# facebookresearch/esm

Measured on AMD Instinct MI355X. Metric: residues/sec (whole node) ESM-2 650M L=1022 bulk extract, higher is better.
Workload: dtype f16; 1 GPU; esm2_t33_650M_UR50D forward (repr_layers=[33] + logits), synthetic tokens [B,1024], random-init weights of the 650M architecture; batch_per_gpu=64, seq_len=1022, ln_fold=on (library default)

## Files before the change

esm_amd/csrc/gemm9.hip:

```cpp
#include "gemm_epi.h"
#include <type_traits>

namespace esmk {

constexpr int Q_BUF = 65536;
constexpr int Q_WOFF = 32768;
constexpr int Q_EPI = 2 * Q_BUF;
constexpr int Q_SLICE = 8192;
constexpr int Q_LDS = Q_EPI + 4 * Q_SLICE;

#define ESMK_INL __attribute__((always_inline))

template <typename T, int EPI, bool FULL, int D = 4, bool NT = true, int NMI = 8, bool SB = false, bool LNF = false>
ESMK_DEV void epilogue9_f32(const GemmArgs& p, f32x4 (&acc)[8][NMI], int m_base, int n_base, int lane, char* wl) {
    static_assert(!LNF || EPI == EPI_RESID_F32, "the LayerNorm-fold producer is the residual epilogue");
    constexpr bool lnp = LNF;
    constexpr int NP = 2 * NMI;
    constexpr int NIB = NMI / 2;
    float s1[4], s2[4];
    float cmv[2][4];
    typedef unsigned u32x2 __attribute__((ext_vector_type(2)));
    typedef unsigned u32x4 __attribute__((ext_vector_type(4)));
    u32x2 hold[4];
    T* h16 = reinterpret_cast<T*>(p.h16);
    if constexpr (!FULL)
        if (n_base >= p.N || m_base >= p.M) return;
    float* out = reinterpret_cast<float*>(p.out);
    const int ldc = p.N;
    const int g4 = lane >> 4, l16 = lane & 15;
    f32x4 old[D][4];
    auto load_old = [&](f32x4 (&dst)[4], int piece) ESMK_INL {
        const int i = piece >> 2, jb = piece & 3;
#pragma unroll
        for (int it = 0; it < 4; ++it) {
            const int pc = it * 64 + lane;
            const int m = FULL ? m_base + 32 * i + (pc >> 3) : min(m_base + 32 * i + (pc >> 3), p.M - 1);
            const int n = FULL ? n_base + 32 * jb + (pc & 7) * 4 : min(n_base + 32 * jb + (pc & 7) * 4, p.N - 4);
            dst[it] = *reinterpret_cast<const f32x4*>(out + (size_t)m * ldc + n);
        }
    };
    if constexpr (EPI == EPI_RESID_F32) {
#pragma unroll
        for (int d = 0; d < D; ++d) load_old(old[d], d);
    }
    auto load_means = [&](int i) ESMK_INL {
#pragma unroll
        for (int it = 0; it < 4; ++it) {
            const int m = m_base + 32 * i + it * 8 + (lane >> 3);
            cmv[i & 1][it] = (kExperiments && (p.lnf_dbg & 4)) ? 0.f : p.ln_mean[FULL ? m : min(m, p.M - 1)];
        }
    };
    if constexpr (LNF)
        if (lnp) load_means(0);
#pragma unroll
    for (int piece = 0; piece < NP; ++piece) {
        const int i = piece >> 2, jb = piece & 3;
        char* sl = wl + (SB ? 0 : (piece & 1) * 4096);
        if constexpr (LNF) {
            if (jb == 0 && lnp) {
#pragma unroll
                for (int it = 0; it < 4; ++it) s1[it] = s2[it] = 0.f;
                if (i + 1 < NIB) load_means(i + 1);
            }
        }
#pragma unroll
        for (int q = 0; q < 4; ++q) {
            const int mi2 = q >> 1, nj2 = q & 1;
            const int row = 16 * mi2 + l16;
            f32x4 v = acc[2 * jb + nj2][2 * i + mi2];
            if constexpr (EPI == EPI_GELU_F32) gelu_fast_x4(v);
            *reinterpret_cast<f32x4*>(sl + row * 128 + (((4 * nj2 + g4) ^ (row & 7)) << 4)) = v;
        }
        f32x4 vv[4];
#pragma unroll
        for (int it = 0; it < 4; ++it) {
            const int pc = it * 64 + lane;
            const int r = pc >> 3, cc = pc & 7;
            vv[it] = *reinterpret_cast<const f32x4*>(sl + r * 128 + ((cc ^ (r & 7)) << 4));
        }
#pragma unroll
        for (int it = 0; it < 4; ++it) {
            const int pc = it * 64 + lane;
            const int r = pc >> 3, cc = pc & 7;
            f32x4 v = vv[it];
            if constexpr (EPI == EPI_RESID_F32) {
                const f32x4 o = old[piece % D][it];
                v = f32x4{o[0] + v[0], o[1] + v[1], o[2] + v[2], o[3] + v[3]};
            }
            const int m = m_base + 32 * i + r, n = n_base + 32 * jb + cc * 4;
            const bool inside = FULL || (m < p.M && n < p.N);
            if (inside) {
                if constexpr (NT) __builtin_nontemporal_store(v, reinterpret_cast<f32x4*>(out + (size_t)m * ldc + n));
                else *reinterpret_cast<f32x4*>(out + (size_t)m * ldc + n) = v;
            }
            if (LNF && lnp) {
                const float c = cmv[i & 1][it];
                float d0 = v[0] - c, d1 = v[1] - c, d2 = v[2] - c, d3 = v[3] - c;
                if (!inside) d0 = d1 = d2 = d3 = 0.f;
                s1[it] += (d0 + d1) + (d2 + d3);
                s2[it] = __builtin_fmaf(d3, d3, __builtin_fmaf(d2, d2, __builtin_fmaf(d1, d1, __builtin_fmaf(d0, d0, s2[it]))));
                typename Op<T>::v4 pk;
                pk[0] = Op<T>::from(d0), pk[1] = Op<T>::from(d1), pk[2] = Op<T>::from(d2), pk[3] = Op<T>::from(d3);
                const u32x2 cur = __builtin_bit_cast(u32x2, pk);
                if ((jb & 1) == 0) {
                    hold[it] = cur;
                } else {
                    const bool odd = (lane & 1) != 0;
                    const u32x2 prev = hold[it];
                    const u32x2 send = odd ? prev : cur;
                    u32x2 recv;
                    recv.x = (unsigned)__builtin_amdgcn_update_dpp(0, (int)send.x, 0xB1, 0xf, 0xf, true);
                    recv.y = (unsigned)__builtin_amdgcn_update_dpp(0, (int)send.y, 0xB1, 0xf, 0xf, true);
                    const u32x4 o = odd ? u32x4{recv.x, recv.y, cur.x, cur.y} : u32x4{prev.x, prev.y, recv.x, recv.y};
                    const int col = n_base + (odd ? 32 * jb + 4 * (cc - 1) : 32 * (jb - 1) + 4 * cc);
                    if ((FULL || (m < p.M && col < p.N)) && !(kExperiments && (p.lnf_dbg & 1))) {
                        auto* hd = reinterpret_cast<u32x4*>(h16 + (size_t)m * p.ldh + col);
                        if constexpr (NT) __builtin_nontemporal_store(o, hd);
                        else *hd = o;
                    }
                }
            }
        }
        if constexpr (EPI == EPI_RESID_F32)
            if (piece + D < NP) load_old(old[piece % D], piece + D);
        if constexpr (LNF) {
            if (jb == 3 && lnp && !(kExperiments && (p.lnf_dbg & 2))) {
#pragma unroll
                for (int it = 0; it < 4; ++it) {
                    float a = s1[it], b = s2[it];
                    a += __builtin_bit_cast(float, __builtin_amdgcn_update_dpp(0, __builtin_bit_cast(int, a), 0x111, 0xf, 0xf, true));
                    b += __builtin_bit_cast(float, __builtin_amdgcn_update_dpp(0, __builtin_bit_cast(int, b), 0x111, 0xf, 0xf, true));
                    a += __builtin_bit_cast(float, __builtin_amdgcn_update_dpp(0, __builtin_bit_cast(int, a), 0x112, 0xf, 0xf, true));
                    b += __builtin_bit_cast(float, __builtin_amdgcn_update_dpp(0, __builtin_bit_cast(int, b), 0x112, 0xf, 0xf, true));
                    a += __builtin_bit_cast(float, __builtin_amdgcn_update_dpp(0, __builtin_bit_cast(int, a), 0x114, 0xf, 0xf, true));
                    b += __builtin_bit_cast(float, __builtin_amdgcn_update_dpp(0, __builtin_bit_cast(int, b), 0x114, 0xf, 0xf, true));
                    const int m = m_base + 32 * i + it * 8 + (lane >> 3);
                    if ((lane & 7) == 7 && (FULL || m < p.M)) {
                        f32x2 st = {a, b};
                        *reinterpret_cast<f32x2*>(p.ln_part + ((size_t)m * p.ln_parts + (n_base >> 7)) * 2) = st;
                    }
                }
            }
        }
    }
}

template <typename T, int EPI, bool FULL, bool NT = false, int NMI = 8, int RR = 32, bool LNF = false, bool X3O = false>
ESMK_DEV void epilogue9_t(const GemmArgs& p, f32x4 (&acc)[8][NMI], int m_base, int n_base, int lane, char* wl) {
    static_assert(!X3O || (EPI == EPI_GELU_T && !LNF), "hi | hi | lo output rows: the plain GELU epilogue");
    using V8 = typename Op<T>::v8;
    float bs1[8], bs2[8];
    constexpr int LPR = EPI == EPI_QKV_ROPE ? 4 : 8;
    constexpr int RPI = 64 / LPR;
    constexpr int NIT = RR / RPI;
    constexpr int NI_ = NMI * 16 / RR;
    float rsv[LNF ? NI_ : 1][NIT];
    if constexpr (LNF) {
        if (FULL || m_base < p.M) {
#pragma unroll
            for (int i = 0; i < NI_; ++i)
#pragma unroll
                for (int it = 0; it < NIT; ++it) {
                    const int m = m_base + RR * i + RPI * it + lane / LPR;
                    rsv[i][it] = p.ln_rstd[FULL ? m : min(m, p.M - 1)];
                }
        }
    }
    constexpr int NI = NMI * 16 / RR;
    constexpr int NR = 2 * NI;
    constexpr int MB = RR / 16;
    const int g4 = lane >> 4, l16 = lane & 15;
    if constexpr (!FULL)
        if (m_base >= p.M) return;
    auto write_round = [&](int r) ESMK_INL {
        const int hf = r / NI, i = r % NI;
#pragma unroll
        for (int mi2 = 0; mi2 < MB; ++mi2)
#pragma unroll
            for (int nq = 0; nq < 4; ++nq) {
                const int row = 16 * mi2 + l16, chunk = 4 * nq + g4;
                *reinterpret_cast<f32x4*>(wl + row * 256 + ((chunk ^ (row & 7)) << 4)) = acc[4 * hf + nq][MB * i + mi2];
            }
    };
    auto read_round = [&](f32x4 (&raw)[8]) ESMK_INL {
        if constexpr (EPI == EPI_QKV_ROPE) {
#pragma unroll
            for (int it = 0; it < RR / 16; ++it) {
                const int slot = it * 64 + lane;
                const int r = slot >> 2, g4 = slot & 3;
#pragma unroll
                for (int e2 = 0; e2 < 2; ++e2) {
                    raw[4 * it + e2] = *reinterpret_cast<const f32x4*>(wl + r * 256 + (((2 * g4 + e2) ^ (r & 7)) << 4));
                    raw[4 * it + 2 + e2] = *reinterpret_cast<const f32x4*>(wl + r * 256 + (((8 + 2 * g4 + e2) ^ (r & 7)) << 4));
                }
            }
        } else {
#pragma unroll
            for (int it = 0; it < RR / 8; ++it) {
                const int slot = it * 64 + lane;
                const int r = slot >> 3, c8 = slot & 7;
#pragma unroll
                for (int e2 = 0; e2 < 2; ++e2)
                    raw[2 * it + e2] = *reinterpret_cast<const f32x4*>(wl + r * 256 + (((2 * c8 + e2) ^ (r & 7)) << 4));
            }
        }
    };
    auto finish_round = [&](int rd, const f32x4 (&raw)[8]) ESMK_INL {
        const int hf = rd / NI, i = rd % NI;
        const int nb = n_base + 64 * hf;
        if constexpr (!FULL)
            if (nb >= p.N) return;
        if constexpr (EPI == EPI_QKV_ROPE) {
            const int which = nb / p.E;
            const int head = (nb - which * p.E) >> 6;
            T* qk = reinterpret_cast<T*>(which == 0 ? p.q : p.k);
            const float sc = which == 0 ? p.scaling : 1.0f;
            if constexpr (LNF) {
                if (i == 0) {
                    const int c0 = nb + 8 * (lane & 3);
#pragma unroll
                    for (int e2 = 0; e2 < 2; ++e2) {
                        f32x4 a = *reinterpret_cast<const f32x4*>(p.bias + c0 + 4 * e2), b = *reinterpret_cast<const f32x4*>(p.bias + c0 + 32 + 4 * e2);
                        if (p.bias2 != nullptr) {
                            const f32x4 a2 = *reinterpret_cast<const f32x4*>(p.bias2 + c0 + 4 * e2), b2 = *reinterpret_cast<const f32x4*>(p.bias2 + c0 + 32 + 4 * e2);
#pragma unroll
                            for (int e = 0; e < 4; ++e) a[e] += a2[e], b[e] += b2[e];
                        }
#pragma unroll
                        for (int e = 0; e < 4; ++e) bs1[4 * e2 + e] = a[e] * sc, bs2[4 * e2 + e] = b[e] * sc;
                    }
                }
            }
#pragma unroll
            for (int it = 0; it < RR / 16; ++it) {
                const int slot = it * 64 + lane;
                const int r = slot >> 2, g4 = slot & 3;
                const int mm = m_base + RR * i + r;
                const int m = FULL ? mm : min(mm, p.M - 1);
                const int b = m / p.T;
                const int tt = p.row_pos != nullptr ? p.row_pos[m] : m - b * p.T;
                float rs = sc;
                if constexpr (LNF) rs = rsv[i][it] * sc;
                float y1[8], y2[8];
#pragma unroll
                for (int e2 = 0; e2 < 2; ++e2) {
                    const f32x4 c = *reinterpret_cast<const f32x4*>(p.cos + (size_t)tt * 32 + 8 * g4 + 4 * e2);
                    const f32x4 s = *reinterpret_cast<const f32x4*>(p.sin + (size_t)tt * 32 + 8 * g4 + 4 * e2);
#pragma unroll
                    for (int e = 0; e < 4; ++e) {
                        const float x1 = LNF ? __builtin_fmaf(raw[4 * it + e2][e], rs, bs1[4 * e2 + e]) : raw[4 * it + e2][e] * sc;
                        const float x2 = LNF ? __builtin_fmaf(raw[4 * it + 2 + e2][e], rs, bs2[4 * e2 + e]) : raw[4 * it + 2 + e2][e] * sc;
                        y1[4 * e2 + e] = __builtin_fmaf(x1, c[e], -(x2 * s[e]));
                        y2[4 * e2 + e] = __builtin_fmaf(x2, c[e], x1 * s[e]);
                    }
                }
                V8 o1, o2;
#pragma unroll
                for (int e = 0; e < 8; ++e) o1[e] = Op<T>::from(y1[e]), o2[e] = Op<T>::from(y2[e]);
                if (FULL || mm < p.M) {
                    T* dst = qk + ((size_t)(b * p.H + head) * p.T + (m - b * p.T)) * 64 + 8 * g4;
                    if constexpr (NT) {
                        __builtin_nontemporal_store(o1, reinterpret_cast<V8*>(dst));
                        __builtin_nontemporal_store(o2, reinterpret_cast<V8*>(dst + 32));
                    } else {
                        *reinterpret_cast<V8*>(dst) = o1;
                        *reinterpret_cast<V8*>(dst + 32) = o2;
                    }
                }
            }
        } else {
            T* out = reinterpret_cast<T*>(p.out);
            if constexpr (LNF) {
                if (i == 0) {
                    const int c0 = FULL ? nb + 8 * (lane & 7) : min(nb + 8 * (lane & 7), p.N - 8);
#pragma unroll
                    for (int e2 = 0; e2 < 2; ++e2) {
                        f32x4 a = *reinterpret_cast<const f32x4*>(p.bias + c0 + 4 * e2);
                        if (p.bias2 != nullptr) {
                            const f32x4 a2 = *reinterpret_cast<const f32x4*>(p.bias2 + c0 + 4 * e2);
#pragma unroll
                            for (int e = 0; e < 4; ++e) a[e] += a2[e];
                        }
#pragma unroll
                        for (int e = 0; e < 4; ++e) bs1[4 * e2 + e] = a[e];
                    }
                }
            }
#pragma unroll
            for (int it = 0; it < RR / 8; ++it) {
                const int slot = it * 64 + lane;
                const int r = slot >> 3, c8 = slot & 7;
                float v[8];
#pragma unroll
                for (int e2 = 0; e2 < 2; ++e2)
#pragma unroll
                    for (int e = 0; e < 4; ++e) v[4 * e2 + e] = raw[2 * it + e2][e];
                if constexpr (LNF) {
                    const float rs = rsv[i][it];
#pragma unroll
                    for (int e = 0; e < 8; ++e) v[e] = __builtin_fmaf(v[e], rs, bs1[e]);
                }
                if constexpr (EPI == EPI_GELU_T) gelu_fast_x8<!X3O>(v);
                V8 o;
#pragma unroll
                for (int e = 0; e < 8; ++e) o[e] = Op<T>::from(v[e]);
                const int m = m_base + RR * i + r, n = nb + 8 * c8;
                if constexpr (X3O) {
                    if (FULL || (m < p.M && n < p.N)) {
                        V8 lo;
#pragma unroll
                        for (int e = 0; e < 8; ++e) lo[e] = Op<T>::from(v[e] - Op<T>::to(o[e]));
                        T* q = out + (size_t)m * (3 * (size_t)p.N) + (size_t)(n >> 6) * 192 + (n & 63);
                        *reinterpret_cast<V8*>(q) = o;
                        *reinterpret_cast<V8*>(q + 64) = o;
                        *reinterpret_cast<V8*>(q + 128) = lo;
                    }
                } else
                if (FULL || (m < p.M && n < p.N)) {
                    if constexpr (NT) __builtin_nontemporal_store(o, reinterpret_cast<V8*>(out + (size_t)m * p.N + n));
                    else *reinterpret_cast<V8*>(out + (size_t)m * p.N + n) = o;
                }
            }
        }
    };
    write_round(0);
#pragma unroll
    for (int rd = 0; rd < NR; ++rd) {
        f32x4 raw[8];
        read_round(raw);
        if (rd + 1 < NR) write_round(rd + 1);
        __builtin_amdgcn_sched_barrier(0);
        finish_round(rd, raw);
    }
}

template <typename T, int EPI, int VAR = 0, bool HM = false, bool LNF = false, bool X3O = false>
__global__ __launch_bounds__(256, 1) void gemm9_kernel(GemmArgs p, unsigned long long* timing) {
    static_assert(!X3O || (EPI == EPI_GELU_T && !HM && !LNF && VAR == 0), "hi | hi | lo output rows: plain full-height GELU kernel");
    static_assert(!LNF || EPI == EPI_RESID_F32 || EPI == EPI_QKV_ROPE || EPI == EPI_V_T || EPI == EPI_GELU_T || EPI == EPI_QKV_ALL,
                  "LayerNorm fold: epilogue");
    constexpr bool LNC = LNF && EPI != EPI_RESID_F32;
    using VtDefault = std::integral_constant<bool, EPI == EPI_V_T>;
    constexpr int TM = HM ? 128 : 256;
    constexpr int NMI = HM ? 4 : 8;
    constexpr int NPC = NMI + 8;
    constexpr int NRD = NMI + 8;
    constexpr int NS = 8 * NMI;
    constexpr int NST = HM ? 3 : 2;
    constexpr int BUF = HM ? 49152 : Q_BUF, WOFF = HM ? 16384 : Q_WOFF;
    constexpr int SLICE = HM ? 4096 : Q_SLICE;
    static_assert(NST * BUF + 4 * SLICE <= Q_LDS, "LDS budget");
    static_assert(!HM || (VAR & ~(8 | 16 | 32 | 64 | 128)) == 0, "half-height tiles: only the timing-experiment bits");
    extern __shared__ __attribute__((aligned(16))) char smem[];
    using V8 = typename Op<T>::v8;
    typedef __attribute__((address_space(3))) void* lds_ptr;
    constexpr bool NO_MFMA = (VAR & 16) != 0, NO_DMA = (VAR & 32) != 0, NO_RD = (VAR & 64) != 0, NO_EPI = (VAR & 128) != 0;
    constexpr int IMODE = VAR & 3;
    constexpr int M_B1 = HM ? 8 : (IMODE == 0 ? 16 : 24);
    constexpr int M_B2 = HM ? 16 : 52;
    constexpr bool STAGGER = (VAR & 4) != 0;
    constexpr bool NO_BAR = (VAR & 8) != 0;
#ifndef ESMK_G9_TIE1
#define ESMK_G9_TIE1 1
#endif
    constexpr bool TIE1 = ESMK_G9_TIE1 && !HM && !NO_MFMA;
    constexpr int KSTAG = (VAR & 256) ? 1 : (VAR & 512) ? 2 : 0;
    constexpr bool HALF_DMA = (VAR & 1024) != 0;
    constexpr int DMA_AUX = (VAR & 2048) ? 2 : 0;
    auto piece_slot = [](int k) constexpr {
        if (HM) return 8 + 2 * k;
        return IMODE == 3 ? 24 + 2 * k : IMODE == 1 ? 24 + k : IMODE == 2 ? 24 + (k * 40) / 16 : 16 + 3 * k;
    };
    auto pieces_before = [piece_slot](int m) constexpr {
        int n = 0;
        for (int k = 0; k < NPC; ++k) n += piece_slot(k) < m ? 1 : 0;
        return n;
    };
    constexpr int IN_FLIGHT0 = pieces_before(M_B2);
    constexpr int IN_FLIGHT = HALF_DMA ? (IN_FLIGHT0 + 1) / 2 : IN_FLIGHT0 + (HM ? NPC : 0);
    const int tid = threadIdx.x;
    const int lane = tid & 63;
    const int wave = __builtin_amdgcn_readfirstlane(tid >> 6);
    const int wr = wave >> 1, wc = wave & 1;
    const int nk = p.K >> 6;
    const unsigned rb = (unsigned)p.K * 2u;
    const unsigned rb_a = p.a_row_bytes ? (unsigned)p.a_row_bytes : rb;
    const bool a_rep = p.a_kt_repeat != 0;

    const int tiles_m = (p.M + TM - 1) / TM, tiles_n = (p.N + 255) >> 8;
    const int total = tiles_m * tiles_n;
    const int xcd = blockIdx.x & 7, slot = blockIdx.x >> 3, nslot = gridDim.x >> 3;
    const int q8 = total >> 3, r8 = total & 7;
    const int start = (xcd < r8) ? xcd * (q8 + 1) : r8 * (q8 + 1) + (xcd - r8) * q8;
    const int cnt = q8 + (xcd < r8 ? 1 : 0);
    const int n_my = (cnt > slot) ? (cnt - slot + nslot - 1) / nslot : 0;
    if (n_my == 0) return;
    const int panel_c = p.panel_c > 0 ? p.panel_c : tiles_n;
    const int panel_full = tiles_m * panel_c;
    auto tile_coords = [&](int it, int& tmi, int& tni) ESMK_INL {
        const int o = start + slot + it * nslot;
        const int pnl = o / panel_full;
        const int rem = o - pnl * panel_full;
        const int w = min(panel_c, tiles_n - pnl * panel_c);
        tmi = __builtin_amdgcn_readfirstlane(rem / w);
        tni = __builtin_amdgcn_readfirstlane(pnl * panel_c + (rem - tmi * w));
    };

    auto uniform_ptr = [](const void* ptr) ESMK_INL {
        const unsigned long long a = (unsigned long long)ptr;
        const unsigned lo = __builtin_amdgcn_readfirstlane((unsigned)a), hi = __builtin_amdgcn_readfirstlane((unsigned)(a >> 32));
        return (void*)(((unsigned long long)hi << 32) | lo);
    };
    __amdgpu_buffer_rsrc_t d_a, d_w;
    int s_kt, s_it;
    unsigned s_koff, s_koff_a;
    const unsigned rb8 = 8u * rb, rb8_a = 8u * rb_a;
    const unsigned vo_base = (unsigned)(64 * wave + (lane >> 3)) * rb;
    const unsigned vo_even = vo_base + (unsigned)(((lane & 7) ^ ((lane >> 4) & 3)) << 4);
    const unsigned vo_odd = vo_base + (unsigned)(((lane & 7) ^ (4 + ((lane >> 4) & 3))) << 4);
    const unsigned va_base = (unsigned)((HM ? 32 : 64) * wave + (lane >> 3)) * rb_a;
    const unsigned va_even = va_base + (unsigned)(((lane & 7) ^ ((lane >> 4) & 3)) << 4);
    const unsigned va_odd = va_base + (unsigned)(((lane & 7) ^ (4 + ((lane >> 4) & 3))) << 4);
    auto set_tile = [&](int it) ESMK_INL {
        int tmi, tni;
        tile_coords(it, tmi, tni);
        s_it = it;
        s_kt = 0;
        if constexpr (KSTAG == 1) s_koff = (unsigned)(((blockIdx.x >> 3) & 3) * (nk >> 2)) * 128u;
        else if constexpr (KSTAG == 2) s_koff = (unsigned)((tni & 3) * (nk >> 2)) * 128u;
        else s_koff = 0;
        s_koff_a = a_rep ? 0u : s_koff;
        const unsigned rows_a = (unsigned)min(TM, p.M - tmi * TM), rows_w = (unsigned)min(256, p.N - tni * 256);
        d_a = __builtin_amdgcn_make_buffer_rsrc(uniform_ptr(reinterpret_cast<const char*>(p.A) + (size_t)tmi * TM * rb_a), 0,
                                                (int)__builtin_amdgcn_readfirstlane(rows_a * rb_a), 0x00020000);
        d_w = __builtin_amdgcn_make_buffer_rsrc(uniform_ptr(reinterpret_cast<const char*>(p.W) + (size_t)tni * 256 * rb), 0,
                                                (int)__builtin_amdgcn_readfirstlane(rows_w * rb), 0x00020000);
    };
    auto advance = [&]() ESMK_INL {
        if (s_kt + 1 < nk) {
            s_kt = s_kt + 1;
            s_koff += 128u;
            if constexpr (KSTAG != 0)
                if (s_koff == (unsigned)nk * 128u) s_koff = 0;
            s_koff_a = a_rep ? (unsigned)(s_kt >> 1) * 128u : s_koff;
        } else if (s_it + 1 < n_my) {
            set_tile(s_it + 1);
        }
    };
    auto issue1 = [&](int k, int buf) ESMK_INL {
        if constexpr (!NO_DMA) {
            if constexpr (HALF_DMA)
                if (k & 1) return;
            const bool isw = HM ? (k >= 4) : ((k & 1) != 0);
            const int q = HM ? (isw ? k - 4 : k) : (k >> 1);
            char* dst = smem + buf * BUF + (isw ? WOFF + wave * 8192 : wave * (HM ? 4096 : 8192)) + q * 1024;
            __builtin_amdgcn_raw_ptr_buffer_load_lds(isw ? d_w : d_a, (lds_ptr)dst, 16,
                                                     isw ? ((q & 1) ? vo_odd : vo_even) : ((q & 1) ? va_odd : va_even),
                                                     isw ? s_koff + (unsigned)q * rb8 : s_koff_a + (unsigned)q * rb8_a, 0, DMA_AUX);
        }
    };

    const int lrow = (lane & 15) * 128;
    const int swz = (lane >> 1) & 7;
    int xo[2];
#pragma unroll
    for (int hf = 0; hf < 2; ++hf) xo[hf] = ((4 * hf + (lane >> 4)) ^ swz) << 4;
    const int a_off = wr * (NMI * 2048) + lrow;
    const int w_off = WOFF + wc * 16384 + lrow;
    V8 xa[NMI], xw[8], ya[NMI], yw[8];
    if constexpr (NO_RD) {
#pragma unroll
        for (int i = 0; i < 8; ++i)
#pragma unroll
            for (int e = 0; e < 8; ++e) {
                xw[i][e] = yw[i][e] = Op<T>::from(0.f);
                if (i < NMI) xa[i][e] = ya[i][e] = Op<T>::from(0.f);
            }
    }
    auto rd1 = [&](V8 (&fa)[NMI], V8 (&fw)[8], const char* bp, int half, int r) ESMK_INL {
        if constexpr (!NO_RD) {
            if (r >= 2 * NMI) {
                const int blk = r - NMI;
                fw[blk] = *reinterpret_cast<const V8*>(bp + w_off + blk * 2048 + xo[half]);
            } else {
                const int blk = r >> 1;
                if (r & 1) fw[blk] = *reinterpret_cast<const V8*>(bp + w_off + blk * 2048 + xo[half]);
                else fa[blk] = *reinterpret_cast<const V8*>(bp + a_off + blk * 2048 + xo[half]);
            }
        }
    };

    f32x4 acc[8][NMI];
    f32x4 bv[8];
    auto load_bias = [&](int n_base) ESMK_INL {
        bool done = false;
        if constexpr (EPI != EPI_V_T && !LNC) {
            bool want = p.bias != nullptr;
            if constexpr (EPI == EPI_QKV_ALL) want = want && n_base < 2 * p.E;
            if (want) {
                const int g4 = lane >> 4;
                if (n_base + 128 <= p.N) {
#pragma unroll
                    for (int nj = 0; nj < 8; ++nj) bv[nj] = *reinterpret_cast<const f32x4*>(p.bias + n_base + 16 * nj + 4 * g4);
                } else {
#pragma unroll
                    for (int nj = 0; nj < 8; ++nj)
#pragma unroll
                        for (int r = 0; r < 4; ++r) {
                            const int n = n_base + 16 * nj + 4 * g4 + r;
                            bv[nj][r] = n < p.N ? p.bias[n] : 0.f;
                        }
                }
                done = true;
            }
        }
        if (!done) {
#pragma unroll
            for (int nj = 0; nj < 8; ++nj) bv[nj] = f32x4{0.f, 0.f, 0.f, 0.f};
        }
    };
    auto mma1 = [&](const V8 (&fa)[NMI], const V8 (&fw)[8], int m, auto first_t, auto vt, auto half_t) ESMK_INL {
        constexpr bool first = decltype(first_t)::value;
        constexpr bool second_half = decltype(half_t)::value;
#pragma unroll
        for (int pp = 0; pp < 2; ++pp) {
            const int idx = 2 * (m % (NS / 2)) + pp;
            const int nj = idx / NMI, mi = idx % NMI;
            f32x4& c = acc[nj][mi];
            const bool use_b = first && m < NS / 2;
            constexpr bool tied = TIE1 && first && second_half;
            if constexpr (NO_MFMA) {
                asm volatile("" ::"v"(fa[mi]), "v"(fw[nj]));
                if (use_b) c = bv[nj];
            } else if constexpr (TIE1 && first) {
                if constexpr (tied) {
                    if constexpr (decltype(vt)::value) Op<T>::mma16_tied(fa[mi], fw[nj], c);
                    else Op<T>::mma16_tied(fw[nj], fa[mi], c);
                } else if constexpr (decltype(vt)::value) {
                    c = Op<T>::mma16(fa[mi], fw[nj], bv[nj]);
                } else {
                    c = Op<T>::mma16(fw[nj], fa[mi], bv[nj]);
                }
            } else if constexpr (decltype(vt)::value) {
                c = use_b ? Op<T>::mma16(fa[mi], fw[nj], bv[nj]) : Op<T>::mma16(fa[mi], fw[nj], c);
            } else {
                c = use_b ? Op<T>::mma16(fw[nj], fa[mi], bv[nj]) : Op<T>::mma16(fw[nj], fa[mi], c);
            }
        }
    };

    int cur = 0;
    auto ktile = [&](auto first, auto vt) ESMK_INL {
        const int nxt = (cur + 1 == NST) ? 0 : cur + 1;
        const char* sb = smem + cur * BUF;
        const char* sn = smem + nxt * BUF;
        advance();
        __builtin_amdgcn_sched_barrier(0);
#pragma unroll
        for (int m = 0; m < NS; ++m) {
            if (m == M_B1) {
                if constexpr (NO_BAR) asm volatile("s_waitcnt lgkmcnt(0)" ::: "memory");
                else asm volatile("s_waitcnt lgkmcnt(0)\n\ts_barrier" ::: "memory");
                __builtin_amdgcn_sched_barrier(0);
            }
            if (m == M_B2) {
                if constexpr (NO_BAR) asm volatile("s_waitcnt vmcnt(%0)" ::"n"(IN_FLIGHT) : "memory");
                else asm volatile("s_waitcnt vmcnt(%0)\n\ts_barrier" ::"n"(IN_FLIGHT) : "memory");
                __builtin_amdgcn_sched_barrier(0);
            }
            if (m < NS / 2) mma1(xa, xw, m, first, vt, std::false_type{});
            else mma1(ya, yw, m, first, vt, std::true_type{});
            if constexpr (HM) {
                if (m < NRD / 2) {
                    rd1(ya, yw, sb, 1, 2 * m);
                    rd1(ya, yw, sb, 1, 2 * m + 1);
                }
            } else {
                if (m < NRD) rd1(ya, yw, sb, 1, m);
            }
            if constexpr (STAGGER) {
                if (m >= M_B1 && m < M_B1 + 32 && ((m - M_B1) & 1) == 0) {
                    if (!(wave & 1)) issue1((m - M_B1) >> 1, cur);
                } else if (m > M_B1 && m < M_B1 + 33 && ((m - M_B1) & 1) == 1) {
                    if (wave & 1) issue1((m - M_B1 - 1) >> 1, cur);
                }
            } else {
#pragma unroll
                for (int k = 0; k < NPC; ++k)
                    if (piece_slot(k) == m) issue1(k, cur);
            }
            if constexpr (M_B2 + NRD <= NS) {
                if (m >= M_B2 && m < M_B2 + NRD) rd1(xa, xw, sn, 0, m - M_B2);
            } else {
                if (m >= M_B2 && m < M_B2 + NRD / 2) {
                    rd1(xa, xw, sn, 0, 2 * (m - M_B2));
                    rd1(xa, xw, sn, 0, 2 * (m - M_B2) + 1);
                }
            }
            __builtin_amdgcn_sched_barrier(0);
        }
        if constexpr (LNF && EPI == EPI_RESID_F32 && !HM) {
#pragma unroll
            for (int nj = 0; nj < 8; ++nj)
#pragma unroll
                for (int mi = 0; mi < NMI; ++mi) asm volatile("" : "+a"(acc[nj][mi]));
        }
        if constexpr (TIE1 && decltype(first)::value) asm volatile("s_nop 7\n\ts_nop 7");
        cur = nxt;
    };

    set_tile(0);
#pragma unroll
    for (int k = 0; k < NPC; ++k) issue1(k, 0);
#pragma unroll
    for (int st = 1; st < NST; ++st) {
        advance();
#pragma unroll
        for (int k = 0; k < NPC; ++k) issue1(k, st);
    }
    if constexpr (EPI == EPI_RESID_F32 && !HM && VAR == 0) {
        if (p.desync > 0) {
            const int g = p.desync_group == 0 ? (int)(blockIdx.x & 1) : p.desync_group == 1 ? (int)((blockIdx.x >> 3) & 1) : (int)(blockIdx.x & 3);
            const long long wait = p.desync_group == 2 ? (long long)g * p.desync / 2 : (long long)g * p.desync;
            if (wait > 0) {
                const unsigned long long t0 = __builtin_readcyclecounter();
                while ((long long)(__builtin_readcyclecounter() - t0) < wait) __builtin_amdgcn_s_sleep(32);
            }
        }
    }
    asm volatile("s_waitcnt vmcnt(%0)\n\ts_barrier" ::"n"(HALF_DMA ? 8 : (NST - 1) * NPC) : "memory");
    __builtin_amdgcn_sched_barrier(0);
#pragma unroll
    for (int r = 0; r < NRD; ++r) rd1(xa, xw, smem, 0, r);

    auto stamp = [&](int it, int k) ESMK_INL {
        if (timing != nullptr && tid == 0) {
            unsigned long long* t = timing + ((size_t)blockIdx.x * 32 + (it & 31)) * 4;
            t[k] = __builtin_readcyclecounter();
            if (k == 2) t[3] = wall_clock64();
        }
    };

    {
        int tmi, tni;
        tile_coords(0, tmi, tni);
        load_bias(tni * 256 + wc * 128);
    }
    for (int it = 0; it < n_my; ++it) {
        int tmi, tni;
        tile_coords(it, tmi, tni);
        constexpr int WRM = TM / 2;
        const int m_base = tmi * TM + wr * WRM, n_base = tni * 256 + wc * 128;
        stamp(it, 0);
        bool v_tile = false;
        if constexpr (EPI == EPI_QKV_ALL) v_tile = tni * 256 >= 2 * p.E;
        if constexpr (EPI == EPI_QKV_ALL) {
            if (v_tile) {
                ktile(std::true_type{}, std::true_type{});
#pragma unroll 1
                for (int kt = 1; kt < nk; ++kt) ktile(std::false_type{}, std::true_type{});
            } else {
                ktile(std::true_type{}, std::false_type{});
#pragma unroll 1
                for (int kt = 1; kt < nk; ++kt) ktile(std::false_type{}, std::false_type{});
            }
        } else {
            ktile(std::true_type{}, VtDefault{});
#pragma unroll 1
            for (int kt = 1; kt < nk; ++kt) ktile(std::false_type{}, VtDefault{});
        }
        stamp(it, 1);
        constexpr bool BIAS_EARLY = (EPI == EPI_STORE_T || EPI == EPI_GELU_T);
        auto next_bias = [&]() ESMK_INL {
            if (it + 1 < n_my) {
                int tm2, tn2;
                tile_coords(it + 1, tm2, tn2);
                load_bias(tn2 * 256 + wc * 128);
            }
        };
        if constexpr (BIAS_EARLY) next_bias();
        char* slice = smem + NST * BUF + wave * SLICE;
        const bool full = (m_base + WRM <= p.M) && (n_base + 128 <= p.N);
        constexpr bool NTS = !HM && (VAR & 4096) == 0;
        if constexpr (NO_EPI) {
#pragma unroll
            for (int nj = 0; nj < 8; ++nj)
#pragma unroll
                for (int mi = 0; mi < NMI; ++mi) asm volatile("" ::"a"(acc[nj][mi]));
        } else if constexpr (EPI == EPI_STORE_F32 || EPI == EPI_GELU_F32 || EPI == EPI_RESID_F32) {
            constexpr int RD = LNF ? 3 : 4;
            if (full) epilogue9_f32<T, EPI, true, RD, NTS, NMI, HM, LNF>(p, acc, m_base, n_base, lane, slice);
            else epilogue9_f32<T, EPI, false, RD, NTS, NMI, HM, LNF>(p, acc, m_base, n_base, lane, slice);
        } else if constexpr (EPI == EPI_V_T) {
#pragma unroll
            for (int hf = 0; hf < 2; ++hf) {
                const int nb = n_base + 64 * hf;
                const bool f2 = (m_base + WRM <= p.M) && (nb + 64 <= p.N) && (p.T % 32 == 0);
                char* sl2 = slice + (HM ? 0 : hf * 4096);
                if (f2) epilogue8m<T, EPI, true, false, false, NMI / 2, 8, NTS, NMI, LNF>(p, acc, 4 * hf, m_base, nb, lane, sl2, 0, 0, 0);
                else epilogue8m<T, EPI, false, false, false, NMI / 2, 8, NTS, NMI, LNF>(p, acc, 4 * hf, m_base, nb, lane, sl2, 0, 0, 0);
            }
        } else if constexpr (EPI == EPI_QKV_ALL) {
            if (v_tile) {
                const int col0 = 2 * p.E;
#pragma unroll
                for (int hf = 0; hf < 2; ++hf) {
                    const int nb = n_base - col0 + 64 * hf;
                    const bool f2 = (m_base + WRM <= p.M) && (nb + 64 <= p.N - col0) && (p.T % 32 == 0);
                    char* sl2 = slice + (HM ? 0 : hf * 4096);
                    if (f2) epilogue8m<T, EPI_V_T, true, false, false, NMI / 2, 8, NTS, NMI, LNF, true>(p, acc, 4 * hf, m_base, nb, lane, sl2, 0, 0, 0, col0);
                    else epilogue8m<T, EPI_V_T, false, false, false, NMI / 2, 8, NTS, NMI, LNF, true>(p, acc, 4 * hf, m_base, nb, lane, sl2, 0, 0, 0, col0);
                }
            } else {
                if (full) epilogue9_t<T, EPI_QKV_ROPE, true, NTS, NMI, HM ? 16 : 32, LNF>(p, acc, m_base, n_base, lane, slice);
                else epilogue9_t<T, EPI_QKV_ROPE, false, NTS, NMI, HM ? 16 : 32, LNF>(p, acc, m_base, n_base, lane, slice);
            }
        } else {
            if (full) epilogue9_t<T, EPI, true, NTS, NMI, HM ? 16 : 32, LNF, X3O>(p, acc, m_base, n_base, lane, slice);
            else epilogue9_t<T, EPI, false, NTS, NMI, HM ? 16 : 32, LNF, X3O>(p, acc, m_base, n_base, lane, slice);
        }
        if constexpr (!BIAS_EARLY) next_bias();
        stamp(it, 2);
    }
    wait_vmcnt0();
}

static unsigned long long* g_timing9 = nullptr;
void gemm9_set_timing(unsigned long long* dev_buf) { g_timing9 = dev_buf; }

static int num_workgroups9() {
    static int n = 0;
    if (n == 0) {
        int dev = 0, cus = 0;
        if (hipGetDevice(&dev) != hipSuccess ||
            hipDeviceGetAttribute(&cus, hipDeviceAttributeMultiprocessorCount, dev) != hipSuccess || cus < 8)
            cus = 256;
        n = cus / 8 * 8;
    }
    return n;
}

template <typename T, int EPI, int VAR = 0, bool HM = false, bool LNF = false, bool X3O = false>
static hipError_t launch9(GemmArgs p, hipStream_t st) {
    static bool attr_set = false;
    auto kern = gemm9_kernel<T, EPI, VAR, HM, LNF, X3O>;
    if (!attr_set) {
        hipError_t e = hipFuncSetAttribute(reinterpret_cast<const void*>(kern),
                                           hipFuncAttributeMaxDynamicSharedMemorySize, Q_LDS);
        if (e != hipSuccess) return e;
        attr_set = true;
    }
    const int tiles_n = (p.N + 255) / 256;
    if (p.panel_c <= 0) {
        if (tiles_n <= 6) p.panel_c = tiles_n;
        else if (tiles_n % 5 == 0) p.panel_c = 5;
        else if (tiles_n % 4 == 0) p.panel_c = 4;
        else if (tiles_n % 6 == 0) p.panel_c = 6;
        else p.panel_c = 5;
    }
    hipLaunchKernelGGL(kern, dim3(num_workgroups9()), dim3(256), Q_LDS, st, p, g_timing9);
    return hipGetLastError();
}

bool gemm9_ln_fold(const GemmArgs& p, int epi) {
    if (epi == EPI_RESID_F32) return p.ln_part != nullptr;
    if (epi == EPI_QKV_ROPE || epi == EPI_V_T || epi == EPI_GELU_T || epi == EPI_QKV_ALL) return p.ln_rstd != nullptr;
    return false;
}

bool gemm9_supports(const GemmArgs& p, int epi) {
    if (p.K % 64 != 0 || p.N % 8 != 0 || p.M <= 0) return false;
    if (p.w_row_bytes || p.a_kt_bytes || p.w_kt_bytes || p.batch > 1 || p.n_valid > 0 || p.ldc > 0 || p.row_keep != nullptr ||
        p.vt_rows > 0 || p.rowmap_R > 0 || epi == EPI_MSA_CTX || p.head_dim != 64)
        return false;
    if (gemm9_ln_fold(p, epi) && p.a_kt_repeat) return false;
    if (p.x3_out && (epi != EPI_GELU_T || p.N % 64 != 0)) return false;
    if (p.a_row_bytes && (p.a_row_bytes % 16 != 0)) return false;
    if ((epi == EPI_QKV_ROPE || epi == EPI_V_T) && p.N % 64 != 0) return false;
    if (epi == EPI_QKV_ALL && !(p.E > 0 && p.E % 128 == 0 && p.N == 3 * p.E && !p.a_kt_repeat && !p.a_row_bytes && p.bias != nullptr))
        return false;
    if ((long long)256 * p.K * 2 > 0x7fffffffLL) return false;
    return (epi >= EPI_STORE_T && epi <= EPI_V_T) || epi == EPI_QKV_ALL;
}

template <typename T>
static hipError_t dispatch9(const GemmArgs& p, int epi, int var, hipStream_t st) {
#ifdef ESMK_EXPERIMENTS
#define ESMK_G9_ALL(V)                                                       \
    switch (epi) {                                                            \
        case EPI_STORE_T: return launch9<T, EPI_STORE_T, V>(p, st);           \
        case EPI_STORE_F32: return launch9<T, EPI_STORE_F32, V>(p, st);       \
        case EPI_GELU_T: return launch9<T, EPI_GELU_T, V>(p, st);             \
        case EPI_GELU_F32: return launch9<T, EPI_GELU_F32, V>(p, st);         \
        case EPI_RESID_F32: return launch9<T, EPI_RESID_F32, V>(p, st);       \
        case EPI_QKV_ROPE: return launch9<T, EPI_QKV_ROPE, V>(p, st);         \
        case EPI_V_T: return launch9<T, EPI_V_T, V>(p, st);                   \
    }
    if (var == 2) { ESMK_G9_ALL(2) }
    if (var == 3) { ESMK_G9_ALL(3) }
#undef ESMK_G9_ALL
    if constexpr (std::is_same<T, _Float16>::value) {
        if (p.half_m > 0 && epi == EPI_STORE_T) {
            switch (var) {
                case 8: return launch9<T, EPI_STORE_T, 8, true>(p, st);
                case 16: return launch9<T, EPI_STORE_T, 16, true>(p, st);
                case 32: return launch9<T, EPI_STORE_T, 32, true>(p, st);
                case 64: return launch9<T, EPI_STORE_T, 64, true>(p, st);
                case 128: return launch9<T, EPI_STORE_T, 128, true>(p, st);
                case 96: return launch9<T, EPI_STORE_T, 96, true>(p, st);
                case 224: return launch9<T, EPI_STORE_T, 224, true>(p, st);
            }
        }
    }
#else
    if (var != 0) return hipErrorInvalidValue;
#endif
    if (p.x3_out) {
        if constexpr (std::is_same<T, _Float16>::value) {
            if (epi == EPI_GELU_T && var == 0 && !gemm9_ln_fold(p, epi)) return launch9<T, EPI_GELU_T, 0, false, false, true>(p, st);
        }
        return hipErrorInvalidValue;
    }
    if (gemm9_ln_fold(p, epi)) {
        if (var != 0) return hipErrorInvalidValue;
        if (epi == EPI_RESID_F32 && (p.h16 == nullptr || p.ln_mean == nullptr || p.ldh < p.N || p.ln_parts < (p.N + 127) / 128))
            return hipErrorInvalidValue;
        if (epi != EPI_RESID_F32 && p.bias == nullptr) return hipErrorInvalidValue;
        if (p.half_m > 0) {
            switch (epi) {
                case EPI_RESID_F32: return launch9<T, EPI_RESID_F32, 0, true, true>(p, st);
                case EPI_QKV_ROPE: return launch9<T, EPI_QKV_ROPE, 0, true, true>(p, st);
                case EPI_V_T: return launch9<T, EPI_V_T, 0, true, true>(p, st);
                case EPI_GELU_T: return launch9<T, EPI_GELU_T, 0, true, true>(p, st);
                case EPI_QKV_ALL: return launch9<T, EPI_QKV_ALL, 0, true, true>(p, st);
            }
        }
        switch (epi) {
            case EPI_RESID_F32: return launch9<T, EPI_RESID_F32, 0, false, true>(p, st);
            case EPI_QKV_ROPE: return launch9<T, EPI_QKV_ROPE, 0, false, true>(p, st);
            case EPI_V_T: return launch9<T, EPI_V_T, 0, false, true>(p, st);
            case EPI_GELU_T: return launch9<T, EPI_GELU_T, 0, false, true>(p, st);
            case EPI_QKV_ALL: return hipErrorInvalidValue;
        }
        return hipErrorInvalidValue;
    }
    if (var == 0 && p.half_m > 0) {
        switch (epi) {
            case EPI_STORE_T: return launch9<T, EPI_STORE_T, 0, true>(p, st);
            case EPI_STORE_F32: return launch9<T, EPI_STORE_F32, 0, true>(p, st);
            case EPI_GELU_T: return launch9<T, EPI_GELU_T, 0, true>(p, st);
            case EPI_GELU_F32: return launch9<T, EPI_GELU_F32, 0, true>(p, st);
            case EPI_RESID_F32: return launch9<T, EPI_RESID_F32, 0, true>(p, st);
            case EPI_QKV_ROPE: return launch9<T, EPI_QKV_ROPE, 0, true>(p, st);
            case EPI_V_T: return launch9<T, EPI_V_T, 0, true>(p, st);
            case EPI_QKV_ALL: return launch9<T, EPI_QKV_ALL, 0, true>(p, st);
        }
    }
    if (var == 0) {
        switch (epi) {
            case EPI_STORE_T: return launch9<T, EPI_STORE_T>(p, st);
            case EPI_STORE_F32: return launch9<T, EPI_STORE_F32>(p, st);
            case EPI_GELU_T: return launch9<T, EPI_GELU_T>(p, st);
            case EPI_GELU_F32: return launch9<T, EPI_GELU_F32>(p, st);
            case EPI_RESID_F32: return launch9<T, EPI_RESID_F32>(p, st);
            case EPI_QKV_ROPE: return launch9<T, EPI_QKV_ROPE>(p, st);
            case EPI_V_T: return launch9<T, EPI_V_T>(p, st);
            case EPI_QKV_ALL: return hipErrorInvalidValue;
        }
    }
#ifdef ESMK_EXPERIMENTS
    if constexpr (std::is_same<T, _Float16>::value) {
        if (epi == EPI_STORE_T) {
            switch (var) {
                case 1: return launch9<T, EPI_STORE_T, 1>(p, st);
                case 7: return launch9<T, EPI_STORE_T, 7>(p, st);
                case 512: return launch9<T, EPI_STORE_T, 512>(p, st);
                case 2048: return launch9<T, EPI_STORE_T, 2048>(p, st);
                case 4096: return launch9<T, EPI_STORE_T, 4096>(p, st);
                case 8: return launch9<T, EPI_STORE_T, 8>(p, st);
                case 16: return launch9<T, EPI_STORE_T, 16>(p, st);
                case 32: return launch9<T, EPI_STORE_T, 32>(p, st);
                case 64: return launch9<T, EPI_STORE_T, 64>(p, st);
                case 128: return launch9<T, EPI_STORE_T, 128>(p, st);
                case 96: return launch9<T, EPI_STORE_T, 96>(p, st);
                case 224: return launch9<T, EPI_STORE_T, 224>(p, st);
                case 1040: return launch9<T, EPI_STORE_T, 1040>(p, st);
            }
        }
    }
#endif
    return hipErrorInvalidValue;
}

hipError_t launch_gemm9(const GemmArgs& p, int epi, int operand_dtype, int var, hipStream_t st) {
    if (!gemm9_supports(p, epi)) return hipErrorInvalidValue;
    if (operand_dtype == ESMK_DT_F16) return dispatch9<_Float16>(p, epi, var, st);
    if (operand_dtype == ESMK_DT_BF16) return dispatch9<__bf16>(p, epi, var, st);
    return hipErrorInvalidValue;
}

}
```

Before: 685,800 residues/s.

## Hoist RoPE index/bias/table loads and add pipelined V-transpose epilogue

The QKV RoPE epilogue now precomputes row positions, output offsets, per-half bias and scaling once per tile. It reorders rounds to interleave the two column halves and prefetches the next cos/sin table rows between rounds, instead of recomputing divisions and reloading tables inside each round. The V-transpose path swaps two calls to the older epilogue8m for a new epilogue9_vt that double-buffers LDS staging rounds and keeps bias and rstd in registers. This adds register pressure and new edge-case code for unaligned T.

```diff
diff --git a/esm_amd/csrc/gemm9.hip b/esm_amd/csrc/gemm9.hip
--- a/esm_amd/csrc/gemm9.hip
+++ b/esm_amd/csrc/gemm9.hip
@@ -149,7 +149,7 @@
 ESMK_DEV void epilogue9_t(const GemmArgs& p, f32x4 (&acc)[8][NMI], int m_base, int n_base, int lane, char* wl) {
     static_assert(!X3O || (EPI == EPI_GELU_T && !LNF), "hi | hi | lo output rows: the plain GELU epilogue");
     using V8 = typename Op<T>::v8;
-    float bs1[8], bs2[8];
+    float bs1[8];
     constexpr int LPR = EPI == EPI_QKV_ROPE ? 4 : 8;
     constexpr int RPI = 64 / LPR;
     constexpr int NIT = RR / RPI;
@@ -172,8 +172,72 @@
     const int g4 = lane >> 4, l16 = lane & 15;
     if constexpr (!FULL)
         if (m_base >= p.M) return;
+    constexpr bool ROPE = EPI == EPI_QKV_ROPE;
+    constexpr int NV = ROPE ? NI * NIT : 1;
+    int rtt[NV];
+    unsigned rro[NV];
+    f32x4 tab[ROPE ? NIT : 1][4];
+    float bsq1[ROPE && LNF ? 2 : 1][8], bsq2[ROPE && LNF ? 2 : 1][8];
+    float sch[2] = {1.0f, 1.0f};
+    T* qkh[2] = {nullptr, nullptr};
+    int headh[2] = {0, 0};
+    auto load_tab = [&](int it, int i) ESMK_INL {
+        const size_t o = (size_t)rtt[i * NIT + it] * 32 + 8 * (lane & 3);
+#pragma unroll
+        for (int e2 = 0; e2 < 2; ++e2) {
+            tab[it][e2] = *reinterpret_cast<const f32x4*>(p.cos + o + 4 * e2);
+            tab[it][2 + e2] = *reinterpret_cast<const f32x4*>(p.sin + o + 4 * e2);
+        }
+    };
+    if constexpr (ROPE) {
+#pragma unroll
+        for (int v = 0; v < NV; ++v) {
+            const int mm = m_base + RR * (v / NIT) + 16 * (v % NIT) + (lane >> 2);
+            const int m = FULL ? mm : min(mm, p.M - 1);
+            const int b = m / p.T;
+            rtt[v] = m - b * p.T;
+            rro[v] = (unsigned)(b * p.H) * (unsigned)p.T + (unsigned)rtt[v];
+        }
+        if (p.row_pos != nullptr) {
+#pragma unroll
+            for (int v = 0; v < NV; ++v) {
+                const int mm = m_base + RR * (v / NIT) + 16 * (v % NIT) + (lane >> 2);
+                rtt[v] = p.row_pos[FULL ? mm : min(mm, p.M - 1)];
+            }
+        }
+#pragma unroll
+        for (int hf = 0; hf < 2; ++hf) {
+            const int nb = n_base + 64 * hf;
+            const bool live = FULL || nb < p.N;
+            const int which = nb / p.E;
+            headh[hf] = (nb - which * p.E) >> 6;
+            qkh[hf] = reinterpret_cast<T*>(which == 0 ? p.q : p.k);
+            sch[hf] = which == 0 ? p.scaling : 1.0f;
+            if constexpr (LNF) {
+                const int c0 = (live ? nb : n_base) + 8 * (lane & 3);
+                f32x4 a[2], b[2];
+#pragma unroll
+                for (int e2 = 0; e2 < 2; ++e2)
+                    a[e2] = *reinterpret_cast<const f32x4*>(p.bias + c0 + 4 * e2), b[e2] = *reinterpret_cast<const f32x4*>(p.bias + c0 + 32 + 4 * e2);
+                if (p.bias2 != nullptr) {
+#pragma unroll
+                    for (int e2 = 0; e2 < 2; ++e2) {
+                        const f32x4 a2 = *reinterpret_cast<const f32x4*>(p.bias2 + c0 + 4 * e2), b2 = *reinterpret_cast<const f32x4*>(p.bias2 + c0 + 32 + 4 * e2);
+#pragma unroll
+                        for (int e = 0; e < 4; ++e) a[e2][e] += a2[e], b[e2][e] += b2[e];
+                    }
+                }
+#pragma unroll
+                for (int e2 = 0; e2 < 2; ++e2)
+#pragma unroll
+                    for (int e = 0; e < 4; ++e) bsq1[hf][4 * e2 + e] = a[e2][e] * sch[hf], bsq2[hf][4 * e2 + e] = b[e2][e] * sch[hf];
+            }
+        }
+#pragma unroll
+        for (int it = 0; it < NIT; ++it) load_tab(it, 0);
+    }
     auto write_round = [&](int r) ESMK_INL {
-        const int hf = r / NI, i = r % NI;
+        const int hf = ROPE ? r % 2 : r / NI, i = ROPE ? r / 2 : r % NI;
 #pragma unroll
         for (int mi2 = 0; mi2 < MB; ++mi2)
 #pragma unroll
@@ -206,59 +270,39 @@
         }
     };
     auto finish_round = [&](int rd, const f32x4 (&raw)[8]) ESMK_INL {
-        const int hf = rd / NI, i = rd % NI;
+        const int hf = ROPE ? rd % 2 : rd / NI, i = ROPE ? rd / 2 : rd % NI;
         const int nb = n_base + 64 * hf;
-        if constexpr (!FULL)
-            if (nb >= p.N) return;
-        if constexpr (EPI == EPI_QKV_ROPE) {
-            const int which = nb / p.E;
-            const int head = (nb - which * p.E) >> 6;
-            T* qk = reinterpret_cast<T*>(which == 0 ? p.q : p.k);
-            const float sc = which == 0 ? p.scaling : 1.0f;
-            if constexpr (LNF) {
-                if (i == 0) {
-                    const int c0 = nb + 8 * (lane & 3);
-#pragma unroll
-                    for (int e2 = 0; e2 < 2; ++e2) {
-                        f32x4 a = *reinterpret_cast<const f32x4*>(p.bias + c0 + 4 * e2), b = *reinterpret_cast<const f32x4*>(p.bias + c0 + 32 + 4 * e2);
-                        if (p.bias2 != nullptr) {
-                            const f32x4 a2 = *reinterpret_cast<const f32x4*>(p.bias2 + c0 + 4 * e2), b2 = *reinterpret_cast<const f32x4*>(p.bias2 + c0 + 32 + 4 * e2);
-#pragma unroll
-                            for (int e = 0; e < 4; ++e) a[e] += a2[e], b[e] += b2[e];
-                        }
-#pragma unroll
-                        for (int e = 0; e < 4; ++e) bs1[4 * e2 + e] = a[e] * sc, bs2[4 * e2 + e] = b[e] * sc;
-                    }
-                }
-            }
-#pragma unroll
-            for (int it = 0; it < RR / 16; ++it) {
-                const int slot = it * 64 + lane;
-                const int r = slot >> 2, g4 = slot & 3;
-                const int mm = m_base + RR * i + r;
-                const int m = FULL ? mm : min(mm, p.M - 1);
-                const int b = m / p.T;
-                const int tt = p.row_pos != nullptr ? p.row_pos[m] : m - b * p.T;
+        if constexpr (ROPE) {
+            const bool live = FULL || nb < p.N;
+            const float sc = sch[hf];
+#pragma unroll
+            for (int it = 0; it < NIT; ++it) {
+                const int g4 = lane & 3;
+                const int mm = m_base + RR * i + 16 * it + (lane >> 2);
                 float rs = sc;
                 if constexpr (LNF) rs = rsv[i][it] * sc;
-                float y1[8], y2[8];
-#pragma unroll
-                for (int e2 = 0; e2 < 2; ++e2) {
-                    const f32x4 c = *reinterpret_cast<const f32x4*>(p.cos + (size_t)tt * 32 + 8 * g4 + 4 * e2);
-                    const f32x4 s = *reinterpret_cast<const f32x4*>(p.sin + (size_t)tt * 32 + 8 * g4 + 4 * e2);
-#pragma unroll
-                    for (int e = 0; e < 4; ++e) {
-                        const float x1 = LNF ? __builtin_fmaf(raw[4 * it + e2][e], rs, bs1[4 * e2 + e]) : raw[4 * it + e2][e] * sc;
-                        const float x2 = LNF ? __builtin_fmaf(raw[4 * it + 2 + e2][e], rs, bs2[4 * e2 + e]) : raw[4 * it + 2 + e2][e] * sc;
-                        y1[4 * e2 + e] = __builtin_fmaf(x1, c[e], -(x2 * s[e]));
-                        y2[4 * e2 + e] = __builtin_fmaf(x2, c[e], x1 * s[e]);
+                V8 o1, o2;
+                if (live) {
+                    float y1[8], y2[8];
+#pragma unroll
+                    for (int e2 = 0; e2 < 2; ++e2) {
+                        const f32x4 c = tab[it][e2], s = tab[it][2 + e2];
+#pragma unroll
+                        for (int e = 0; e < 4; ++e) {
+                            const float x1 = LNF ? __builtin_fmaf(raw[4 * it + e2][e], rs, bsq1[LNF ? hf : 0][4 * e2 + e]) : raw[4 * it + e2][e] * sc;
+                            const float x2 = LNF ? __builtin_fmaf(raw[4 * it + 2 + e2][e], rs, bsq2[LNF ? hf : 0][4 * e2 + e]) : raw[4 * it + 2 + e2][e] * sc;
+                            y1[4 * e2 + e] = __builtin_fmaf(x1, c[e], -(x2 * s[e]));
+                            y2[4 * e2 + e] = __builtin_fmaf(x2, c[e], x1 * s[e]);
+                        }
                     }
-                }
-                V8 o1, o2;
-#pragma unroll
-                for (int e = 0; e < 8; ++e) o1[e] = Op<T>::from(y1[e]), o2[e] = Op<T>::from(y2[e]);
-                if (FULL || mm < p.M) {
-                    T* dst = qk + ((size_t)(b * p.H + head) * p.T + (m - b * p.T)) * 64 + 8 * g4;
+#pragma unroll
+                    for (int e = 0; e < 8; ++e) o1[e] = Op<T>::from(y1[e]), o2[e] = Op<T>::from(y2[e]);
+                }
+                __builtin_amdgcn_sched_barrier(0);
+                if (hf == 1 && i + 1 < NI) load_tab(it, i + 1);
+                __builtin_amdgcn_sched_barrier(0);
+                if (live && (FULL || mm < p.M)) {
+                    T* dst = qkh[hf] + ((size_t)rro[i * NIT + it] + (size_t)headh[hf] * p.T) * 64 + 8 * g4;
                     if constexpr (NT) {
                         __builtin_nontemporal_store(o1, reinterpret_cast<V8*>(dst));
                         __builtin_nontemporal_store(o2, reinterpret_cast<V8*>(dst + 32));
@@ -269,6 +313,8 @@
                 }
             }
         } else {
+            if constexpr (!FULL)
+                if (nb >= p.N) return;
             T* out = reinterpret_cast<T*>(p.out);
             if constexpr (LNF) {
                 if (i == 0) {
@@ -327,6 +373,136 @@
 #pragma unroll
     for (int rd = 0; rd < NR; ++rd) {
         f32x4 raw[8];
+        read_round(raw);
+        if (rd + 1 < NR) write_round(rd + 1);
+        __builtin_amdgcn_sched_barrier(0);
+        finish_round(rd, raw);
+    }
+}
+
+template <typename T, bool FULL, bool NT, int NMI, bool LNF, bool COL0>
+ESMK_DEV void epilogue9_vt(const GemmArgs& p, f32x4 (&acc)[8][NMI], int m_base, int n_base, int lane, char* wl, int col0) {
+    using V8 = typename Op<T>::v8;
+    constexpr int NTH = NMI / 4;
+    constexpr int CH = NMI == 8 ? 32 : 16;
+    constexpr int NCG = 128 / CH;
+    constexpr int NR = NTH * NCG;
+    constexpr int NIT = CH / 8;
+    const int g4 = lane >> 4, l16 = lane & 15;
+    const int c8 = lane & 7, r8 = lane >> 3;
+    const int ncols = COL0 ? p.N - col0 : p.N;
+    if constexpr (!FULL)
+        if (m_base >= p.M || n_base >= ncols) return;
+    T* vt = reinterpret_cast<T*>(p.vt);
+    const bool aligned = FULL || (p.T % 32 == 0);
+    float bvc[NCG][NIT];
+#pragma unroll
+    for (int cg = 0; cg < NCG; ++cg)
+#pragma unroll
+        for (int it = 0; it < NIT; ++it) {
+            const int n = n_base + CH * cg + 8 * it + r8;
+            bvc[cg][it] = p.bias[(COL0 ? col0 : 0) + (FULL ? n : min(n, ncols - 1))];
+        }
+    if constexpr (LNF) {
+        if (p.bias2 != nullptr) {
+#pragma unroll
+            for (int cg = 0; cg < NCG; ++cg)
+#pragma unroll
+                for (int it = 0; it < NIT; ++it) {
+                    const int n = n_base + CH * cg + 8 * it + r8;
+                    bvc[cg][it] += p.bias2[(COL0 ? col0 : 0) + (FULL ? n : min(n, ncols - 1))];
+                }
+        }
+    }
+    f32x4 rs[LNF ? NTH : 1][2];
+    if constexpr (LNF) {
+#pragma unroll
+        for (int th = 0; th < NTH; ++th)
+#pragma unroll
+            for (int e2 = 0; e2 < 2; ++e2)
+                rs[th][e2] = *reinterpret_cast<const f32x4*>(p.ln_rstd + m_base + 64 * th + 16 * (c8 >> 1) + 4 * ((c8 & 1) + 2 * e2));
+    }
+    size_t run[NTH];
+#pragma unroll
+    for (int th = 0; th < NTH; ++th) {
+        const int m = m_base + 64 * th + 8 * c8;
+        const int mc = FULL ? m : min(m, p.M - 1);
+        const int b = mc / p.T;
+        run[th] = (size_t)(b * p.H * 64) * p.Tp + (mc - b * p.T);
+    }
+    auto write_round = [&](int r) ESMK_INL {
+        const int th = r / NCG, cg = r % NCG;
+#pragma unroll
+        for (int nj2 = 0; nj2 < CH / 16; ++nj2)
+#pragma unroll
+            for (int mq = 0; mq < 4; ++mq) {
+                const int row = 16 * nj2 + l16, chunk = 4 * mq + g4;
+                *reinterpret_cast<f32x4*>(wl + row * 256 + ((chunk ^ (row & 7)) << 4)) = acc[(CH / 16) * cg + nj2][4 * th + mq];
+            }
+    };
+    auto read_round = [&](f32x4 (&raw)[2 * NIT]) ESMK_INL {
+#pragma unroll
+        for (int it = 0; it < NIT; ++it) {
+            const int r = 8 * it + r8;
+#pragma unroll
+            for (int e2 = 0; e2 < 2; ++e2)
+                raw[2 * it + e2] = *reinterpret_cast<const f32x4*>(wl + r * 256 + (((4 * (c8 >> 1) + (c8 & 1) + 2 * e2) ^ (r & 7)) << 4));
+        }
+    };
+    size_t eo[8];
+    auto finish_round = [&](int rd, const f32x4 (&raw)[2 * NIT]) ESMK_INL {
+        const int th = rd / NCG, cg = rd % NCG;
+        if constexpr (!FULL) {
+            if (n_base + CH * cg >= ncols) return;
+            if (!aligned && cg == 0) {
+#pragma unroll
+                for (int e2 = 0; e2 < 2; ++e2)
+#pragma unroll
+                    for (int e = 0; e < 4; ++e) {
+                        const int m = m_base + 64 * th + 16 * (c8 >> 1) + 4 * ((c8 & 1) + 2 * e2) + e;
+                        const int mc = min(m, p.M - 1);
+                        const int b = mc / p.T, t = mc - b * p.T;
+                        const int t16 = t & 15;
+                        const int tp = (t & ~15) | ((((t16 >> 2) & 1) << 3) | (((t16 >> 3) & 1) << 2) | (t16 & 3));
+                        eo[4 * e2 + e] = m < p.M ? (size_t)(b * p.H * 64) * p.Tp + tp : ~(size_t)0;
+                    }
+            }
+        }
+#pragma unroll
+        for (int it = 0; it < NIT; ++it) {
+            const int n = n_base + CH * cg + 8 * it + r8;
+            const float bv = bvc[cg][it];
+            float x[8];
+#pragma unroll
+            for (int e2 = 0; e2 < 2; ++e2)
+#pragma unroll
+                for (int e = 0; e < 4; ++e) {
+                    if constexpr (LNF) x[4 * e2 + e] = __builtin_fmaf(raw[2 * it + e2][e], rs[th][e2][e], bv);
+                    else x[4 * e2 + e] = raw[2 * it + e2][e] + bv;
+                }
+            asm volatile("" : "+v"(x[0]), "+v"(x[1]), "+v"(x[2]), "+v"(x[3]), "+v"(x[4]), "+v"(x[5]), "+v"(x[6]), "+v"(x[7]));
+            V8 o;
+#pragma unroll
+            for (int e = 0; e < 8; ++e) o[e] = Op<T>::from(x[e]);
+            if (aligned) {
+                if (FULL || (m_base + 64 * th + 8 * c8 < p.M && n < ncols)) {
+                    T* dst = vt + run[th] + (size_t)n * p.Tp;
+                    if constexpr (NT) __builtin_nontemporal_store(o, reinterpret_cast<V8*>(dst));
+                    else *reinterpret_cast<V8*>(dst) = o;
+                }
+            } else if constexpr (!FULL) {
+                if (n < ncols) {
+#pragma unroll
+                    for (int e = 0; e < 8; ++e)
+                        if (eo[e] != ~(size_t)0) vt[eo[e] + (size_t)n * p.Tp] = o[e];
+                }
+            }
+        }
+    };
+    write_round(0);
+#pragma unroll
+    for (int rd = 0; rd < NR; ++rd) {
+        f32x4 raw[2 * NIT];
         read_round(raw);
         if (rd + 1 < NR) write_round(rd + 1);
         __builtin_amdgcn_sched_barrier(0);
@@ -692,25 +868,13 @@
             if (full) epilogue9_f32<T, EPI, true, RD, NTS, NMI, HM, LNF>(p, acc, m_base, n_base, lane, slice);
             else epilogue9_f32<T, EPI, false, RD, NTS, NMI, HM, LNF>(p, acc, m_base, n_base, lane, slice);
         } else if constexpr (EPI == EPI_V_T) {
-#pragma unroll
-            for (int hf = 0; hf < 2; ++hf) {
-                const int nb = n_base + 64 * hf;
-                const bool f2 = (m_base + WRM <= p.M) && (nb + 64 <= p.N) && (p.T % 32 == 0);
-                char* sl2 = slice + (HM ? 0 : hf * 4096);
-                if (f2) epilogue8m<T, EPI, true, false, false, NMI / 2, 8, NTS, NMI, LNF>(p, acc, 4 * hf, m_base, nb, lane, sl2, 0, 0, 0);
-                else epilogue8m<T, EPI, false, false, false, NMI / 2, 8, NTS, NMI, LNF>(p, acc, 4 * hf, m_base, nb, lane, sl2, 0, 0, 0);
-            }
+            if (full && p.T % 32 == 0) epilogue9_vt<T, true, NTS, NMI, LNF, false>(p, acc, m_base, n_base, lane, slice, 0);
+            else epilogue9_vt<T, false, NTS, NMI, LNF, false>(p, acc, m_base, n_base, lane, slice, 0);
         } else if constexpr (EPI == EPI_QKV_ALL) {
             if (v_tile) {
                 const int col0 = 2 * p.E;
-#pragma unroll
-                for (int hf = 0; hf < 2; ++hf) {
-                    const int nb = n_base - col0 + 64 * hf;
-                    const bool f2 = (m_base + WRM <= p.M) && (nb + 64 <= p.N - col0) && (p.T % 32 == 0);
-                    char* sl2 = slice + (HM ? 0 : hf * 4096);
-                    if (f2) epilogue8m<T, EPI_V_T, true, false, false, NMI / 2, 8, NTS, NMI, LNF, true>(p, acc, 4 * hf, m_base, nb, lane, sl2, 0, 0, 0, col0);
-                    else epilogue8m<T, EPI_V_T, false, false, false, NMI / 2, 8, NTS, NMI, LNF, true>(p, acc, 4 * hf, m_base, nb, lane, sl2, 0, 0, 0, col0);
-                }
+                if (full && p.T % 32 == 0) epilogue9_vt<T, true, NTS, NMI, LNF, true>(p, acc, m_base, n_base - col0, lane, slice, col0);
+                else epilogue9_vt<T, false, NTS, NMI, LNF, true>(p, acc, m_base, n_base - col0, lane, slice, col0);
             } else {
                 if (full) epilogue9_t<T, EPI_QKV_ROPE, true, NTS, NMI, HM ? 16 : 32, LNF>(p, acc, m_base, n_base, lane, slice);
                 else epilogue9_t<T, EPI_QKV_ROPE, false, NTS, NMI, HM ? 16 : 32, LNF>(p, acc, m_base, n_base, lane, slice);
```

New measurement: 696,500 residues/s, median of 6. +1.6%, better.
